# jcmgray/cotengra

Measured on NVIDIA H100. Metric: sycamore_n53_m20_sliced_contract_tflops, higher is better.
Workload: dtype c128 (f64 arithmetic)

## Files before the change

cotengra_b200/csrc/absorbdot.cuh:

```cuda
#pragma once

constexpr int AB_STAGES = 4;
constexpr int AB_THREADS = 256;
constexpr int AB_VSTAGE = 2 * 32 * 32;
constexpr int AB_ASTAGE = 2 * 32 * 16;
constexpr size_t AB_SMEM = (size_t)(128 * 16 + AB_STAGES * (AB_VSTAGE + AB_ASTAGE)) * sizeof(double2);

__device__ __forceinline__ double ab_neg(double x) { return __longlong_as_double(__double_as_longlong(x) ^ (1ll << 63)); }

__global__ void __launch_bounds__(AB_THREADS, 1)
absorbdot_kernel(const int64_t* __restrict__ D, const double2* __restrict__ A, const double2* __restrict__ Bs,
                 const double2* __restrict__ V, double2* __restrict__ C) {
  extern __shared__ __align__(16) double2 ab_smem[];
  double2* sB = ab_smem;
  double2* sV = sB + 128 * 16;
  double2* sA = sV + AB_STAGES * AB_VSTAGE;
  __shared__ long long t_ma[32], t_mc[32], t_nv[32], t_cv[128], t_ka[16];

  const int tid = threadIdx.x, lane = tid & 31, warp = tid >> 5;
  const int N = (int)D[AB_N], K = (int)D[AB_K], CC = (int)D[AB_C], CCP = (int)D[AB_CCP], KL = (int)D[AB_KL];
  const int NG = (int)D[AB_NG];
  const long long kla = D[AB_KLA], klv = D[AB_KLV];
  for (int i = tid; i < 32; i += AB_THREADS) {
    t_ma[i] = D[AB_TMA + i];
    t_mc[i] = D[AB_TMC + i];
    t_nv[i] = D[AB_TNV + i];
  }
  for (int i = tid; i < 128; i += AB_THREADS) t_cv[i] = D[AB_TCV + i];
  for (int i = tid; i < 16; i += AB_THREADS) t_ka[i] = D[AB_TKA + i];
  for (int i = tid; i < 128 * 16; i += AB_THREADS) {
    const int c = i >> 4, k = i & 15;
    const long long cb = D[AB_TCB + c];
    const bool ok = cb >= 0 && k < K;
    cp_async_zfill<16>(sB + c * 16 + (k ^ ((c & 1) << 2)), ok ? Bs + D[AB_TKB + k] + cb : Bs, ok);
  }
  __syncthreads();

  const unsigned long long U = (unsigned long long)D[AB_UNITS];
  const unsigned u0 = (unsigned)(U * blockIdx.x / gridDim.x), u1 = (unsigned)(U * (blockIdx.x + 1) / gridDim.x);
  const int nq = CCP >> 5;
  const long long nstage = (long long)(u1 - u0) * nq;

  unsigned g_ext = 1, g_div = 1;
  long long g_sa = 0, g_sv = 0;
  if (lane < NG) {
    g_ext = (unsigned)D[AB_G + lane * 4];
    g_div = (unsigned)D[AB_G + lane * 4 + 1];
    g_sa = D[AB_G + lane * 4 + 2];
    g_sv = D[AB_G + lane * 4 + 3];
  }
  auto unit_base = [&](unsigned u, long long& oa, long long& ov) {
    const long long dgt = (long long)((u / g_div) % g_ext);
    long long a = dgt * g_sa, v = dgt * g_sv;
#pragma unroll
    for (int o = 16; o > 0; o >>= 1) {
      a += __shfl_xor_sync(0xffffffffu, a, o);
      v += __shfl_xor_sync(0xffffffffu, v, o);
    }
    oa = a;
    ov = v;
  };

  unsigned lu = u0;
  int lq = 0;
  long long la = 0, lv = 0;
  if (nstage > 0) unit_base(lu, la, lv);
  long long issued = 0;
  auto issue = [&]() {
    if (issued < nstage) {
      const int slot = (int)(issued % AB_STAGES);
      double2* dv = sV + slot * AB_VSTAGE;
      double2* da = sA + slot * AB_ASTAGE;
#pragma unroll
      for (int j = 0; j < 8; ++j) {
        const int e = j * AB_THREADS + tid, cq = e & 31, kl = (e >> 5) & 1, n = e >> 6, c = lq * 32 + cq;
        const bool ok = kl < KL && n < N && c < CC;
        cp_async_zfill<16>(dv + (kl * 32 + n) * 32 + (cq ^ (n & 1)), ok ? V + lv + kl * klv + t_nv[n] + t_cv[c] : V, ok);
      }
#pragma unroll
      for (int j = 0; j < 4; ++j) {
        const int e = j * AB_THREADS + tid, k = e & 15, kl = (e >> 4) & 1, m = e >> 5;
        const bool ok = k < K && kl < KL && t_mc[m] >= 0;
        cp_async_zfill<16>(da + (kl * 32 + m) * 16 + (k ^ ((m & 1) << 2)), ok ? A + la + kl * kla + t_ka[k] + t_ma[m] : A,
                           ok);
      }
      ++issued;
      if (++lq == nq) {
        lq = 0;
        ++lu;
        if (issued < nstage) unit_base(lu, la, lv);
      }
    }
    cp_async_commit();
  };
#pragma unroll 1
  for (int s = 0; s < AB_STAGES - 1; ++s) issue();

  const int g = lane >> 2, t = lane & 3;
  const int wmh = warp >> 2, wcb = warp & 3;
  int bofs[2];
#pragma unroll
  for (int i = 0; i < 2; ++i) bofs[i] = (int)D[AB_TBCK + 2 * wmh + i] * CCP * 16;
  double Rr[4][2][2], Ri[4][2][2];
#pragma unroll
  for (int nb = 0; nb < 4; ++nb)
#pragma unroll
    for (int i = 0; i < 2; ++i) Rr[nb][i][0] = Rr[nb][i][1] = Ri[nb][i][0] = Ri[nb][i][1] = 0.0;

#pragma unroll 1
  for (long long s = 0; s < nstage; ++s) {
    cp_async_wait<AB_STAGES - 2>();
    __syncthreads();
    issue();
    const int slot = (int)(s % AB_STAGES), q = (int)(s % nq);
    if (q * 32 + wcb * 8 >= CC) continue;
    const double2* vb = sB + (q * 32 + wcb * 8 + g) * 16;
#pragma unroll
    for (int kl = 0; kl < 2; ++kl) {
      if (kl >= KL) break;
      const double2* va = sA + slot * AB_ASTAGE + (kl * 32 + wmh * 16) * 16;
      const double2* vv = sV + slot * AB_VSTAGE + kl * 32 * 32;
      double Xr[2][2], Xi[2][2];
#pragma unroll
      for (int i = 0; i < 2; ++i) Xr[i][0] = Xr[i][1] = Xi[i][0] = Xi[i][1] = 0.0;
#pragma unroll
      for (int ks = 0; ks < 4; ++ks) {
        const int kk = (ks * 4 + t) ^ ((g & 1) << 2);
#pragma unroll
        for (int i = 0; i < 2; ++i) {
          const double2 b = vb[bofs[i] + kk];
          const double2 a = va[(i * 8 + g) * 16 + kk];
          dmma16x8x4(Xr[i], Xi[i], a.x, a.y, b.x);
          dmma16x8x4(Xr[i], Xi[i], ab_neg(a.y), a.x, b.y);
        }
      }
#pragma unroll
      for (int p = 0; p < 2; ++p) {
#pragma unroll
        for (int nb = 0; nb < 4; ++nb) {
          const double2 v = vv[(nb * 8 + g) * 32 + ((wcb * 8 + 2 * t + p) ^ (g & 1))];
          const double nvi = ab_neg(v.y);
#pragma unroll
          for (int i = 0; i < 2; ++i) {
            dmma16x8x4(Rr[nb][i], Ri[nb][i], v.x, v.y, Xr[i][p]);
            dmma16x8x4(Rr[nb][i], Ri[nb][i], nvi, v.x, Xi[i][p]);
          }
        }
      }
    }
  }
  cp_async_wait<0>();
  __syncthreads();

  double2* red = sV;
#pragma unroll
  for (int nb = 0; nb < 4; ++nb)
#pragma unroll
    for (int i = 0; i < 2; ++i)
#pragma unroll
      for (int e = 0; e < 2; ++e)
        red[wcb * 1024 + ((2 * wmh + i) * 8 + 2 * t + e) * 32 + nb * 8 + g] = make_double2(Rr[nb][i][e], Ri[nb][i][e]);
  __syncthreads();
  for (int i = tid; i < 1024; i += AB_THREADS) {
    const int m = i >> 5, n = i & 31;
    if (t_mc[m] < 0 || n >= N) continue;
    double2 sum = red[i];
#pragma unroll
    for (int w = 1; w < 4; ++w) sum = add_of(sum, red[w * 1024 + i]);
    atomic_add_of(C + t_mc[m] + D[AB_TNC + n], sum);
  }
}
```

cotengra_b200/csrc/ctg_b200.cu:

```cuda
#include <cuda.h>
#include <cuda_runtime.h>
#include <stdint.h>
#include <stdio.h>
#include <stdlib.h>
#include <string.h>

#include <algorithm>
#include <atomic>
#include <type_traits>
#include <string>
#include <vector>

#include "../../include/ctg_b200.h"
#include "gett_desc.h"
#include "gett_kernels.cuh"
#include "probe.cuh"

using namespace ctgb;

namespace {

thread_local std::string g_err;
std::atomic<int64_t> g_launches{0};

// ... 233 lines not shown
  if (!di.ok) return fail(CTGB_E_CUDA, "no CUDA device");
  DsLaunch lc;
  if (int rc = dmmastream_launch_config(h, di.sms, lc)) return rc;
  if (lc.blocks == 0) return CTGB_OK;
  const bool strip = desc_stripped(h);
  const double2 *a = (const double2*)A, *b = (const double2*)B;
  double2* c = (double2*)C;
  const unsigned blocks = (unsigned)lc.blocks;
  switch (lc.nj) {
    case 1: dmmastream_launch<1, 4>(strip, blocks, d, a, b, c, st); break;
    case 2: dmmastream_launch<2, 4>(strip, blocks, d, a, b, c, st); break;
    case 4: dmmastream_launch<4, 4>(strip, blocks, d, a, b, c, st); break;
    default: dmmastream_launch<8, 2>(strip, blocks, d, a, b, c, st); break;
  }
  g_launches.fetch_add(1, std::memory_order_relaxed);
  CUDA_TRY(cudaGetLastError());
  return CTGB_OK;
}

int launch_absorb_root(const int64_t* h, const int64_t* d, const void* A, const void* Bs, const void* V, void* C,
                       cudaStream_t st) {
  if (h[W_DTYPE] != CTGB_C128) return fail(CTGB_E_VALUE, "the absorb-root kernel is complex128 only");
  if (h[AB_M] < 1 || h[AB_M] > 32 || h[AB_N] < 1 || h[AB_N] > 32 || h[AB_K] < 1 || h[AB_K] > 16 || h[AB_C] < 1 ||
      h[AB_C] > h[AB_CCP] || h[AB_CCP] % 32 || h[AB_CCP] > 128 || (h[AB_KL] != 1 && h[AB_KL] != 2) || h[AB_NG] < 0 || h[AB_NG] > AB_MAXG || h[AB_UNITS] < 1 || h[AB_UNITS] >= (1ll << 32) ||
      h[AB_GRID] < 1 || h[AB_GRID] > h[AB_UNITS] || h[AB_GRID] > (1 << 20))
    return fail(CTGB_E_VALUE, "absorb-root descriptor out of range");
  for (int mb = 0; mb < 4; ++mb)
    if (h[AB_TBCK + mb] < 0 || (h[AB_TBCK + mb] + 1) * h[AB_CCP] > 128)
      return fail(CTGB_E_VALUE, "absorb-root descriptor out of range");
  if (!(h[W_FLAGS] & 1)) {
    if (h[W_CELEMS] <= 0) return fail(CTGB_E_VALUE, "absorb-root into a strided C needs accumulate");
    CUDA_TRY(cudaMemsetAsync(C, 0, (size_t)h[W_CELEMS] * sizeof(double2), st));
  }
  static bool attr = false;
  if (!attr) {
    CUDA_TRY(cudaFuncSetAttribute(absorbdot_kernel, cudaFuncAttributeMaxDynamicSharedMemorySize, (int)AB_SMEM));
    attr = true;
  }
  absorbdot_kernel<<<(unsigned)h[AB_GRID], AB_THREADS, AB_SMEM, st>>>(d, (const double2*)A, (const double2*)Bs,
                                                                      (const double2*)V, (double2*)C);
  g_launches.fetch_add(1, std::memory_order_relaxed);
  CUDA_TRY(cudaGetLastError());
  return CTGB_OK;
}

std::atomic<int64_t> g_tmap_launches{0};

struct Tc05Box {
  int nb = 0;
  struct Dim { uint64_t ext, stride; } dim[8];
};
int tc05_tensor_map_box(const int64_t* h, uint64_t a_addr, Tc05Box& bx) {
  if (a_addr & 15u) return 0;
  auto& box = bx.dim;
  int& nb = bx.nb;
  nb = 0;
  const int n_lda = (int)h[W_NLDA];
  for (int i = 0; i < n_lda; ++i) {
    const uint64_t ext = (uint64_t)h[OFF_LDA + 4 * i], st = (uint64_t)h[OFF_LDA + 4 * i + 1];
    if (h[OFF_LDA + 4 * i + 1] <= 0) return 0;
    if (nb && st == box[nb - 1].stride * box[nb - 1].ext) {
      box[nb - 1].ext *= ext;
    } else {
      if (nb == 4) return 0;
      box[nb].ext = ext;
      box[nb].stride = st;
      ++nb;
    }
  }
  for (int i = 0; i < nb; ++i) {
    while (box[i].ext > 256) {
      uint64_t f = 256;
      while (f > 1 && box[i].ext % f) --f;
// ... 1074 lines not shown
```

cotengra_b200/executor.py:

```python

from __future__ import annotations

import ctypes as C
import math

import numpy as np

from . import _lib, lowering
from .lowering import (
    DTYPE_CODES,
    DTYPE_SIZES,
    accumulator_dtype,
    build_pair_desc,
    build_single_desc,
    check_precision,
    check_tensordot_shapes,
    classify_pair,
    classify_single,
    dtype_name,
    row_major_strides,
    split_equation,
    tensordot_terms,
)

# ... 199 lines not shown
        if self.acc_dtype not in (None, self.dtype):
            _lib.check(lib.ctgb_plan_set_accumulator(h, DTYPE_CODES[self.acc_dtype]))
        if self.scale_slots is not None:
            n = len(self.nodes)
            sa, sb = ((C.c_int32 * max(n, 1))(*s) for s in self.scale_slots)
            _lib.check(lib.ctgb_plan_set_scale_slots(h, sa, sb, n))
        return self

    def destroy(self):
        if self.handle is not None:
            _lib.load().ctgb_plan_destroy(self.handle)
            self.handle = None

    def launches_per_slice(self):
        return int(_lib.load().ctgb_plan_launches_per_slice(self.handle))

    def strip_modes(self):
        n = len(self.nodes)
        pre, after = (C.c_int32 * n)(), (C.c_int32 * n)()
        _lib.check(_lib.load().ctgb_plan_strip_modes(self.handle, pre, after, n))
        return [(int(a), int(b)) for a, b in zip(pre, after)]

    def __del__(self):
        try:
            self.destroy()
        except Exception:
            pass


class ExecPlan(_DevicePlan):

    def __init__(self, contractions, inputs, output, size_dict, sliced=(), dtype="complex128",
                 strip_exponent=False, hoist=True, allow_dmma=True, sm_count=None,
                 variant=None, precision="3xtf32", accumulate="native", absorb_root=False):
        self.dtype = dtype_name(dtype)
        self.precision = check_precision(precision, self.dtype)
        self.esize = DTYPE_SIZES[self.dtype]
        self.acc_dtype = accumulator_dtype(self.dtype, accumulate)
        self.wide = self.acc_dtype != self.dtype
        self.contractions = tuple(contractions)
        self.inputs = [tuple(t) for t in inputs]
        self.output = tuple(output)
        self.size_dict = dict(size_dict)
        self.sliced = [(i, int(s), None if p is None else int(p)) for i, s, p in sliced]
        self.strip_exponent = bool(strip_exponent)
        if sm_count is None:
            try:
                sm_count = _lib.device_info()["sm_count"]
            except Exception:
                sm_count = 132
        self.sm_count = sm_count
        self.absorb_root = bool(absorb_root) and self.dtype == "complex128" and not self.strip_exponent \
            and variant is None
        self._build(hoist, allow_dmma, variant)

    def _build(self, hoist, allow_dmma, variant):
        sliced_pos = {ind: j for j, (ind, _s, _p) in enumerate(self.sliced)}
        nslices = math.prod(s for _i, s, p in self.sliced if p is None)
        self.nslices = nslices
        real_slicing = bool(self.sliced)
        hoist = hoist and real_slicing

        def out_ext(ix):
            if ix in sliced_pos and self.sliced[sliced_pos[ix]][2] is not None:
                return 1
            return self.size_dict[ix]

        self.out_shape = tuple(out_ext(ix) for ix in self.output)
        out_full_strides = row_major_strides(self.out_shape)
        self.out_elements = math.prod(self.out_shape)
        root_term = tuple(ix for ix in self.output if ix not in sliced_pos)
        root_strides = [s for ix, s in zip(self.output, out_full_strides) if ix not in sliced_pos]
        self.root_shape = tuple(self.size_dict[ix] for ix in root_term)
        self.slice_out_stride = [0] * len(self.sliced)
        for ix, s in zip(self.output, out_full_strides):
            if ix in sliced_pos and self.sliced[sliced_pos[ix]][2] is None:
                self.slice_out_stride[sliced_pos[ix]] += s

        cur = {}
        self.input_nbytes = []
        for i, term in enumerate(self.inputs):
            full_shape = [self.size_dict[ix] for ix in term]
            fs = row_major_strides(full_shape)
            self.input_nbytes.append(math.prod(full_shape) * self.esize)
            keep = [k for k, ix in enumerate(term) if ix not in sliced_pos]
            cut = [k for k, ix in enumerate(term) if ix in sliced_pos]
            cur[i] = _Slot([full_shape[k] for k in keep], [fs[k] for k in keep], K_INPUT, self.input_nbytes[-1],
# ... 11 lines not shown
                terms, out = split_equation(arg)
                if len(terms) != 1:
                    raise ValueError(f"expected a single-term equation, got {arg!r}")
                is_root = l is not None
                if is_root and not is_last:
                    raise ValueError("single-input record must be the only contraction")
                ostr = root_strides if (is_root and direct) else None
                odims, sdims, oshape = classify_single(terms[0], src.shape, out, out_strides=ostr,
                                                      strides_x=src.strides)
                if is_root:
                    self._check_root_shape(oshape)
                acc = is_root and direct
                words = build_single_desc(odims, sdims, self.dtype, accumulate=acc)
                dst = _Slot(oshape, row_major_strides(oshape), K_SCRATCH, max(math.prod(oshape), 1) * self.esize,
                            variant=src.variant)
                nodes.append(dict(kind=1, a=src, b=None, c=dst, words=words, root=is_root))
                tensors.append(dst)
                cur[p] = dst
                continue

            A, Bt = cur.pop(l), cur.pop(r)
            if tdot:
                axes = (tuple(arg[0]), tuple(arg[1]))
                check_tensordot_shapes(axes, A.shape, Bt.shape)
                ta, tb, to = tensordot_terms(axes, len(A.shape), len(Bt.shape), perm)
            else:
                terms, to = split_equation(arg)
                if len(terms) != 2:
                    raise ValueError(f"expected a two-term equation, got {arg!r}")
                ta, tb = terms
            is_root = is_last

            def lower(into_output, wide_c=False):
                ostr = root_strides if into_output else None
                dims = classify_pair(ta, A.shape, tb, Bt.shape, to, out_strides=ostr,
                                     strides_a=A.strides, strides_b=Bt.strides)
                dense = 0 if into_output else math.prod(dims.out_shape)
                return dims, dense, build_pair_desc(dims, self.dtype, accumulate=into_output,
                                                    sm_count=self.sm_count, allow_dmma=allow_dmma,
                                                    c_dense_elems=dense, variant=variant,
                                                    precision=self.precision, wide_c=wide_c)

            if is_root and self.wide and not self.strip_exponent:
                direct = lower(True)[2].variant in lowering.DOTSTREAM_VARIANTS
                dims, dense, plan = lower(direct, wide_c=direct)
            else:
                dims, dense, plan = lower(is_root and direct)
            if is_root:
                self._check_root_shape(dims.out_shape)
            acc = is_root and direct
            dst = _Slot(dims.out_shape, row_major_strides(dims.out_shape), K_SCRATCH,
                        max(math.prod(dims.out_shape), 1) * self.esize, variant=A.variant or Bt.variant)
            a, b = (Bt, A) if plan.swapped else (A, Bt)
            nodes.append(dict(kind=0, a=a, b=b, c=dst, words=plan.words, root=is_root, plan=plan,
                              sizes=plan.sizes, dims=dims, acc=acc, dense=dense, terms=(A, Bt)))
            tensors.append(dst)
            cur[p] = dst
            if self.absorb_root:
                self._absorb(nodes, tensors)

        if not nodes:
            raise ValueError("empty contraction program")
        self.root_direct = direct
        if direct:
            nodes[-1]["c"].kind = K_OUTPUT
        for nd in nodes:
            srcs = [t for t in (nd["a"], nd["b"], nd.get("d")) if t is not None]
            nd["invariant"] = bool(hoist and not nd["root"] and not any(s.variant for s in srcs))
            nd["phase"] = PHASE_INV_FWD if nd["invariant"] else PHASE_VAR_FWD
            if nd["invariant"]:
                nd["c"].kind = K_PERSISTENT
            else:
                nd["c"].variant = True
        order = [nd for nd in nodes if nd["invariant"]] + [nd for nd in nodes if not nd["invariant"]]
        for pos, nd in enumerate(order):
            nd["pos"] = pos
        self.workspace_bytes, self.persistent_bytes, _ = layout(order)
        self.nodes = nodes
        self.n_variant_nodes = sum(1 for nd in nodes if not nd["invariant"])

        self.macs_per_slice = 0
        self.macs_invariant = 0
        self.elements_per_slice = 0
        for nd in nodes:
            if nd["kind"] != 0:
                continue
            macs = nd["plan"].macs if nd.get("d") is not None else math.prod(nd["sizes"])
            el = sum(math.prod(nd[x].shape) for x in ("a", "b", "d", "c") if nd.get(x) is not None)
            if nd["invariant"]:
                self.macs_invariant += macs
            else:
                self.macs_per_slice += macs
                self.elements_per_slice += el

        self.tensors = tensors
        self._marshal()
        if not direct:
            rs = self.root_shape
            dense = row_major_strides(rs)
            odims = [[e, sx, so] for e, sx, so in zip(rs, dense, root_strides) if e != 1]
            self._chunk_words = build_single_desc(odims, [], self.dtype)

    def _absorb(self, nodes, tensors):
        if len(nodes) < 2:
            return
        P, R = nodes[-2], nodes[-1]
        if P["kind"] != 0 or R["kind"] != 0 or P.get("d") is not None or R["plan"].variant != lowering.VAR_DMMA_32x32:
            return
        X = P["c"]
        if X not in R["terms"]:
            return
        ab = lowering.build_absorb_desc(P["dims"], R["dims"], R["terms"][0] is X, accumulate=R["acc"],
                                        sm_count=self.sm_count, c_dense_elems=R["dense"])
        if ab is None:
            return
        pa, pb = P["terms"]
        small, big = (pa, pb) if ab.small_is_a else (pb, pa)
        V = R["terms"][1] if R["terms"][0] is X else R["terms"][0]
        tensors.remove(X)
        nodes[-2:] = [dict(kind=0, a=big, b=V, d=small, c=R["c"], words=ab.words, root=R["root"], plan=ab,
                           sizes=ab.sizes, dims=None, acc=R["acc"], dense=R["dense"], terms=None)]

    def _check_root_shape(self, shape):
        if tuple(shape) != tuple(self.root_shape):
            raise ValueError(
                f"contraction program produces shape {tuple(shape)}, "
                f"tree output expects {tuple(self.root_shape)}"
            )

    def host_staging_bytes(self):
        extra = _align(self.total_bytes) - self.total_bytes
        for n in self.input_nbytes:
            extra += _align(n)
        return extra + _align(self.out_elements * DTYPE_SIZES[self.acc_dtype]) + 512

    def execute(self, input_ptrs, out_ptr, exp_ptr, ws_ptr, ws_bytes, begin, step, count, stream=0):
        lib = _lib.load()
        arr = (C.c_void_p * len(input_ptrs))(*input_ptrs)
        _lib.check(lib.ctgb_plan_execute(self.handle, arr, out_ptr, exp_ptr, None, None, ws_ptr, ws_bytes,
                                         int(begin), int(step), int(count), stream))

    def execute_host(self, host_arrays, host_out, ws_ptr, ws_bytes, begin, step, count, stream=0):
        lib = _lib.load()
        ptrs = (C.c_void_p * len(host_arrays))(*[a.ctypes.data for a in host_arrays])
        nb = (C.c_int64 * len(host_arrays))(*[a.nbytes for a in host_arrays])
        exp = C.c_double(0.0)
        _lib.check(lib.ctgb_plan_execute_host(self.handle, ptrs, nb, host_out.ctypes.data,
                                              C.byref(exp), ws_ptr, ws_bytes, int(begin), int(step),
                                              int(count), stream))
        return exp.value

    def profile(self, enable=True):
        _lib.check(_lib.load().ctgb_plan_profile(self.handle, int(enable)))

# ... 6 lines not shown
```

cotengra_b200/lowering.py:

```python

from __future__ import annotations

import math
from collections import Counter, namedtuple
from dataclasses import dataclass, field

import numpy as np

MAX_T, MAX_G, MAX_GB, MAX_LD = 12, 40, 12, 24
(W_MAGIC, W_DTYPE, W_NTM, W_NTN, W_NTK, W_NGM, W_NGN, W_NGK, W_NGB, W_MTA,
 W_NTA, W_KTA, W_TILES_M, W_TILES_N, W_TILES_B, W_STEPS_K, W_SPLITK, W_PGM,
 W_MFULL, W_MTEXT, W_MW, W_PGN, W_NFULL, W_NTEXT, W_NW, W_PGK, W_KFULL,
 W_KTEXT, W_KW, W_NLDA, W_NLDB, W_FLAGS, W_VARIANT, W_CELEMS, W_RUNA, W_LBOPAD) = range(36)
W_HDR = 40
OFF_TM = W_HDR
OFF_TN = OFF_TM + MAX_T * 3
OFF_TK = OFF_TN + MAX_T * 3
OFF_GM = OFF_TK + MAX_T * 3
OFF_GN = OFF_GM + MAX_G * 4
OFF_GK = OFF_GN + MAX_G * 4
OFF_GB = OFF_GK + MAX_G * 4
OFF_LDA = OFF_GB + MAX_GB * 5
OFF_LDB = OFF_LDA + MAX_LD * 4
DESC_WORDS = OFF_LDB + MAX_LD * 4
# ... 555 lines not shown
    for off, rows, width in ((OFF_TM, t.tm, 3), (OFF_TN, t.tn, 3), (OFF_TK, t.tk, 3), (OFF_GM, t.gm, 4),
                             (OFF_GN, t.gn, 4), (OFF_GK, t.gk, 4), (OFF_GB, t.gb, 5), (OFF_LDA, t.lda, 4),
                             (OFF_LDB, t.ldb, 4)):
        for i, r in enumerate(rows):
            W[off + i * width: off + (i + 1) * width] = r
    return W




AB_M, AB_N, AB_K, AB_C, AB_KL, AB_NG, AB_UNITS, AB_KLA, AB_KLV, AB_GRID, AB_BS_SLOT, AB_CCP = range(2, 14)
AB_MAXG = 32
AB_TMA = W_HDR
AB_TMC, AB_TNV, AB_TNC = AB_TMA + 32, AB_TMA + 64, AB_TMA + 96
AB_TKA = AB_TMA + 128
AB_TKB = AB_TKA + 16
AB_TCB = AB_TKB + 16
AB_TCV = AB_TCB + 128
AB_G = AB_TCV + 128
AB_TBCK = AB_G + AB_MAXG * 4


@dataclass
class AbsorbPlan:

    words: np.ndarray
    small_is_a: bool
    sizes: tuple
    macs: int
    variant: int = VAR_ABSORB_ROOT
    swapped: bool = False
    splitk: int = 1
    tiles: int = 1


def _enum(dims, cols):
    out = [[0] for _ in cols]
    for d in dims:
        out = [[o + i * d[c] for i in range(d[0]) for o in lst] for lst, c in zip(out, cols)]
    return out


def build_absorb_desc(dp: PairDims, dr: PairDims, x_is_a, accumulate=False, sm_count=132, c_dense_elems=0):
    if dp.batch or dr.batch:
        return None
    xi = 1 if x_is_a else 2
    vi = 3 - xi
    r_keep = {d[xi]: (d[0], d[3]) for d in (dr.m if x_is_a else dr.n)}
    v_keep = [[d[0], d[vi], d[3]] for d in (dr.n if x_is_a else dr.m)]
    r_con = {d[xi]: (d[0], d[vi]) for d in dr.k}
    if len(r_con) != len(dr.k) or len(r_keep) != len(dr.m if x_is_a else dr.n):
        return None
    for small_is_a in (False, True):
        small = dp.m if small_is_a else dp.n
        big = dp.n if small_is_a else dp.m
        bi, si = (2, 1) if small_is_a else (1, 2)
        xdims = {d[3]: d for d in small + big}
        if not small or len(xdims) != len(small) + len(big) or set(xdims) != set(r_keep) | set(r_con):
            continue
        if any(xdims[x][0] != (r_keep.get(x) or r_con[x])[0] for x in xdims):
            continue
        small_x = {d[3] for d in small}
        rows = [[d[0], d[bi], r_keep[d[3]][1]] for d in big if d[3] in r_keep]
        ck = [[d[0], d[si], r_keep[d[3]][1]] for d in small if d[3] in r_keep]
        cc = sorted(([d[0], d[si], r_con[d[3]][1]] for d in small if d[3] in r_con), key=lambda d: d[2])
        kprime = [[d[0], d[bi], r_con[d[3]][1]] for d in big if d[3] in r_con]
        MX, CK = math.prod(d[0] for d in rows), math.prod(d[0] for d in ck)
        N, K, CC = math.prod(d[0] for d in v_keep), math.prod(d[0] for d in dp.k), math.prod(d[0] for d in cc)
        CCP = -(-CC // 32) * 32
        rows_per = 8 if CK > 1 else 32
        if MX > rows_per or CK * rows_per > 32 or N > 32 or K > 16 or CK * CCP > 128 or not small_x:
            return None
        kl = min(kprime, key=lambda d: d[2], default=None)
        if kl is not None and kl[0] == 2:
            kprime.remove(kl)
        else:
            kl = [1, 0, 0]
        grid = sorted(kprime, key=lambda d: (d[1], d[2]))
        if len(grid) > AB_MAXG:
            return None
        units = math.prod(d[0] for d in grid)
        w = np.zeros(DESC_WORDS, dtype=np.int64)
        w[0], w[1] = DESC_MAGIC, DTYPE_CODES["complex128"]
        w[AB_M], w[AB_N], w[AB_K], w[AB_C], w[AB_CCP], w[AB_KL] = CK * rows_per if CK > 1 else MX, N, K, CC, CCP, kl[0]
        w[AB_NG], w[AB_UNITS], w[AB_KLA], w[AB_KLV] = len(grid), units, kl[1], kl[2]
        w[AB_GRID] = min(units, sm_count)
        w[AB_BS_SLOT] = -1
        w[W_FLAGS] = int(bool(accumulate))
        w[W_VARIANT] = VAR_ABSORB_ROOT
        w[W_CELEMS] = c_dense_elems
        ra, rc = _enum(rows, (1, 2))
        ckb, ckc = _enum(ck, (1, 2))
        ma, mc = [-1] * 32, [-1] * 32
        for j, (ob, oc) in enumerate(zip(ckb, ckc)):
            for r, (a, c) in enumerate(zip(ra, rc)):
                ma[j * rows_per + r], mc[j * rows_per + r] = a, c + oc
        tbck = [min(mb * 8 // rows_per, CK - 1) for mb in range(4)]
        nv, nc = _enum(v_keep, (1, 2))
        ka, kb = _enum([[d[0], d[bi], d[si]] for d in dp.k], (1, 2))
        cb, cv = _enum(cc, (1, 2))
        tcb = [-1] * 128
        for j, ob in enumerate(ckb):
            tcb[j * CCP:j * CCP + CC] = [ob + o for o in cb]
        for off, vals in ((AB_TMA, ma), (AB_TMC, mc), (AB_TNV, nv), (AB_TNC, nc), (AB_TKA, ka), (AB_TKB, kb),
                          (AB_TCB, tcb), (AB_TCV, cv), (AB_TBCK, tbck)):
            w[off:off + len(vals)] = vals
        div = 1
        for j, (e, sa, sv) in enumerate(grid):
            w[AB_G + 4 * j:AB_G + 4 * j + 4] = (e, div, sa, sv)
            div *= e
        kp = units * kl[0]
        M = MX * CK
        return AbsorbPlan(w, small_is_a, (1, M, N, kp * CC), MX * kp * K * CC * CK + M * N * kp * CC)
    return None


def classify_single(term, shape, out, out_strides=None, strides_x=None):
    term, out = tuple(term), tuple(out)
    shape = tuple(map(int, shape))
    if len(term) != len(shape):
        raise ValueError(f"Term '{term}' does not match shape {shape}.")
    sx = row_major_strides(shape) if strides_x is None else list(strides_x)
    ext, st_x, order = {}, {}, []
    for ix, d, s in zip(term, shape, sx):
        if ix not in order:
            order.append(ix)
        if ext.setdefault(ix, d) != d:
            raise ValueError(f"Index {ix} has mismatched sizes {ext[ix]} and {d}.")
        st_x[ix] = st_x.get(ix, 0) + s
    for ix in out:
        if ix not in ext:
            raise ValueError(f"Output index {ix} does not appear in the input.")
    out_shape = tuple(ext[ix] for ix in out)
    so = row_major_strides(out_shape) if out_strides is None else list(out_strides)
    odims = [[ext[ix], st_x[ix], s] for ix, s in zip(out, so) if ext[ix] != 1]
    sdims = [[ext[ix], st_x[ix]] for ix in order if ix not in out and ext[ix] != 1]
    return odims, sdims, out_shape


def build_single_desc(odims, sdims, dtype, accumulate=False) -> np.ndarray:
    dtype = dtype_name(dtype)
    odims = coalesce(odims)
    sdims = coalesce(sdims)
    odims.sort(key=lambda d: abs(d[2]) if d[2] else 1 << 62)
    sdims.sort(key=lambda d: abs(d[1]) if d[1] else 1 << 62)
    if len(odims) > MAX_S or len(sdims) > MAX_S:
        raise NotImplementedError("too many dims for a single-operand node")
# ... 26 lines not shown
```

cotengra_b200/csrc/gett_kernels.cuh:

```cuda
#pragma once
#include <cuda_runtime.h>
#include <math_constants.h>
#include <stdint.h>

#include <type_traits>

#include "gett_desc.h"

namespace ctgb {

__device__ __forceinline__ void mac(float& c, float a, float b) { c = fmaf(a, b, c); }
__device__ __forceinline__ void mac(double& c, double a, double b) { c = fma(a, b, c); }
__device__ __forceinline__ void mac(float2& c, float2 a, float2 b) {
  c.x = fmaf(a.x, b.x, c.x);
  c.x = fmaf(-a.y, b.y, c.x);
  c.y = fmaf(a.x, b.y, c.y);
  c.y = fmaf(a.y, b.x, c.y);
}
__device__ __forceinline__ void mac(double2& c, double2 a, double2 b) {
  c.x = fma(a.x, b.x, c.x);
  c.x = fma(-a.y, b.y, c.x);
  c.y = fma(a.x, b.y, c.y);
  c.y = fma(a.y, b.x, c.y);
}
// ... 497 lines not shown
    for (int i = 0; i < FM; ++i)
#pragma unroll
      for (int j = 0; j < FN; ++j) {
        if constexpr (TR) {
          const int r = (wm * FM + i) * 8 + fc;
          const int c = (wn * FN + j) * 8 + frow;
          store(r, c, make_double2(acc.re[i][j][0], acc.im[i][j][0]));
          store(r + 1, c, make_double2(acc.re[i][j][1], acc.im[i][j][1]));
          continue;
        }
        const int r = (wm * FM + i) * 8 + frow;
        const int c = (wn * FN + j) * 8 + fc;
        if constexpr (CPLX) {
          if (pair_ok) {
            store_pair(r, c, make_double2(acc.re[i][j][0], acc.im[i][j][0]),
                       make_double2(acc.re[i][j][1], acc.im[i][j][1]));
          } else {
            store(r, c, make_double2(acc.re[i][j][0], acc.im[i][j][0]));
            store(r, c + 1, make_double2(acc.re[i][j][1], acc.im[i][j][1]));
          }
        } else {
          store(r, c, acc.re[i][j][0]);
          store(r, c + 1, acc.re[i][j][1]);
        }
      }
  }
};

#include "tf32_policy.cuh"
#include "stream_rows.cuh"
#include "rowstream.cuh"
#include "dmmastream.cuh"
#include "dotstream.cuh"
#include "absorbdot.cuh"
#include "tc05_policy.cuh"
#include "gett_ws.cuh"
#include "tc05_kernel.cuh"

template <typename T>
__global__ void single_kernel(const int64_t* __restrict__ D, const T* __restrict__ X, T* __restrict__ out) {
  const int n_o = (int)D[S_NO], n_s = (int)D[S_NS];
  const long long out_elems = D[S_OUT_ELEMS], sum_elems = D[S_SUM_ELEMS];
  const bool accumulate = (D[S_FLAGS] & 1) != 0;
  for (long long o = blockIdx.x * (long long)blockDim.x + threadIdx.x; o < out_elems;
       o += (long long)gridDim.x * blockDim.x) {
    long long e = o, xo = 0, oo = 0;
    for (int d = 0; d < n_o; ++d) {
      const int64_t* L = D + OFF_SO + d * 3;
      long long dig = e % L[0];
      e /= L[0];
      xo += dig * L[1];
      oo += dig * L[2];
    }
    T acc = zero_of<T>();
    for (long long s = 0; s < sum_elems; ++s) {
      long long e2 = s, xs = 0;
      for (int d = 0; d < n_s; ++d) {
        const int64_t* L = D + OFF_SS + d * 2;
        xs += (e2 % L[0]) * L[1];
        e2 /= L[0];
      }
      acc = add_of(acc, X[xo + xs]);
    }
    out[oo] = accumulate ? add_of(out[oo], acc) : acc;
  }
}

template <typename T>
__global__ void __launch_bounds__(256) single_reduce_kernel(const int64_t* __restrict__ D, const T* __restrict__ X,
// ... 182 lines not shown
```

Baseline: 24.38.

## Template absorb-root kernel on row count and add optional block-friendly root layout

The absorb-root kernel is now templated on whether the A rows collapse to 8 unique rows. When they do, it loads a smaller A tile per stage and uses a deeper 5-stage cp.async ring. The host checks the row tables to pick the instantiation. Separately, a new opt-in root_layout option rewrites the output strides of the producer steps feeding the absorbed root, so A and V arrive in a block-friendly bit order. That option is off by default and adds a second build pass when enabled.

```diff
diff --git a/cotengra_b200/csrc/absorbdot.cuh b/cotengra_b200/csrc/absorbdot.cuh
--- a/cotengra_b200/csrc/absorbdot.cuh
+++ b/cotengra_b200/csrc/absorbdot.cuh
@@ -1,16 +1,23 @@
 #pragma once
 
-constexpr int AB_STAGES = 4;
 constexpr int AB_THREADS = 256;
 constexpr int AB_VSTAGE = 2 * 32 * 32;
-constexpr int AB_ASTAGE = 2 * 32 * 16;
-constexpr size_t AB_SMEM = (size_t)(128 * 16 + AB_STAGES * (AB_VSTAGE + AB_ASTAGE)) * sizeof(double2);
+template <bool ROWS8>
+struct AbRing {
+  static constexpr int STAGES = ROWS8 ? 5 : 4;
+  static constexpr int AROWS = ROWS8 ? 8 : 32;
+  static constexpr int ASTAGE = 2 * AROWS * 16;
+  static constexpr size_t SMEM = (size_t)(128 * 16 + STAGES * (AB_VSTAGE + ASTAGE)) * sizeof(double2);
+};
+static_assert(AbRing<true>::SMEM <= 232448 && AbRing<false>::SMEM <= 232448, "absorb-root ring fits shared memory");
 
 __device__ __forceinline__ double ab_neg(double x) { return __longlong_as_double(__double_as_longlong(x) ^ (1ll << 63)); }
 
+template <bool ROWS8>
 __global__ void __launch_bounds__(AB_THREADS, 1)
 absorbdot_kernel(const int64_t* __restrict__ D, const double2* __restrict__ A, const double2* __restrict__ Bs,
                  const double2* __restrict__ V, double2* __restrict__ C) {
+  constexpr int AB_STAGES = AbRing<ROWS8>::STAGES, AB_AROWS = AbRing<ROWS8>::AROWS, AB_ASTAGE = AbRing<ROWS8>::ASTAGE;
   extern __shared__ __align__(16) double2 ab_smem[];
   double2* sB = ab_smem;
   double2* sV = sB + 128 * 16;
@@ -78,11 +85,11 @@
         cp_async_zfill<16>(dv + (kl * 32 + n) * 32 + (cq ^ (n & 1)), ok ? V + lv + kl * klv + t_nv[n] + t_cv[c] : V, ok);
       }
 #pragma unroll
-      for (int j = 0; j < 4; ++j) {
+      for (int j = 0; j < AB_AROWS / 8; ++j) {
         const int e = j * AB_THREADS + tid, k = e & 15, kl = (e >> 4) & 1, m = e >> 5;
         const bool ok = k < K && kl < KL && t_mc[m] >= 0;
-        cp_async_zfill<16>(da + (kl * 32 + m) * 16 + (k ^ ((m & 1) << 2)), ok ? A + la + kl * kla + t_ka[k] + t_ma[m] : A,
-                           ok);
+        cp_async_zfill<16>(da + (kl * AB_AROWS + m) * 16 + (k ^ ((m & 1) << 2)),
+                           ok ? A + la + kl * kla + t_ka[k] + t_ma[m] : A, ok);
       }
       ++issued;
       if (++lq == nq) {
@@ -118,7 +125,7 @@
 #pragma unroll
     for (int kl = 0; kl < 2; ++kl) {
       if (kl >= KL) break;
-      const double2* va = sA + slot * AB_ASTAGE + (kl * 32 + wmh * 16) * 16;
+      const double2* va = sA + slot * AB_ASTAGE + (kl * AB_AROWS + (ROWS8 ? 0 : wmh * 16)) * 16;
       const double2* vv = sV + slot * AB_VSTAGE + kl * 32 * 32;
       double Xr[2][2], Xi[2][2];
 #pragma unroll
@@ -129,7 +136,7 @@
 #pragma unroll
         for (int i = 0; i < 2; ++i) {
           const double2 b = vb[bofs[i] + kk];
-          const double2 a = va[(i * 8 + g) * 16 + kk];
+          const double2 a = va[((ROWS8 ? 0 : i * 8) + g) * 16 + kk];
           dmma16x8x4(Xr[i], Xi[i], a.x, a.y, b.x);
           dmma16x8x4(Xr[i], Xi[i], ab_neg(a.y), a.x, b.y);
         }
diff --git a/cotengra_b200/csrc/ctg_b200.cu b/cotengra_b200/csrc/ctg_b200.cu
--- a/cotengra_b200/csrc/ctg_b200.cu
+++ b/cotengra_b200/csrc/ctg_b200.cu
@@ -289,13 +289,22 @@
     if (h[W_CELEMS] <= 0) return fail(CTGB_E_VALUE, "absorb-root into a strided C needs accumulate");
     CUDA_TRY(cudaMemsetAsync(C, 0, (size_t)h[W_CELEMS] * sizeof(double2), st));
   }
-  static bool attr = false;
-  if (!attr) {
-    CUDA_TRY(cudaFuncSetAttribute(absorbdot_kernel, cudaFuncAttributeMaxDynamicSharedMemorySize, (int)AB_SMEM));
-    attr = true;
-  }
-  absorbdot_kernel<<<(unsigned)h[AB_GRID], AB_THREADS, AB_SMEM, st>>>(d, (const double2*)A, (const double2*)Bs,
-                                                                      (const double2*)V, (double2*)C);
+  bool rows8 = true;
+  for (int r = 8; r < 32; ++r)
+    if (h[AB_TMC + r] >= 0 && (h[AB_TMC + (r & 7)] < 0 || h[AB_TMA + r] != h[AB_TMA + (r & 7)])) rows8 = false;
+  static bool attr[2] = {false, false};
+  if (!attr[rows8]) {
+    CUDA_TRY(cudaFuncSetAttribute(rows8 ? absorbdot_kernel<true> : absorbdot_kernel<false>,
+                                  cudaFuncAttributeMaxDynamicSharedMemorySize,
+                                  (int)(rows8 ? AbRing<true>::SMEM : AbRing<false>::SMEM)));
+    attr[rows8] = true;
+  }
+  if (rows8)
+    absorbdot_kernel<true><<<(unsigned)h[AB_GRID], AB_THREADS, AbRing<true>::SMEM, st>>>(
+        d, (const double2*)A, (const double2*)Bs, (const double2*)V, (double2*)C);
+  else
+    absorbdot_kernel<false><<<(unsigned)h[AB_GRID], AB_THREADS, AbRing<false>::SMEM, st>>>(
+        d, (const double2*)A, (const double2*)Bs, (const double2*)V, (double2*)C);
   g_launches.fetch_add(1, std::memory_order_relaxed);
   CUDA_TRY(cudaGetLastError());
   return CTGB_OK;
diff --git a/cotengra_b200/executor.py b/cotengra_b200/executor.py
--- a/cotengra_b200/executor.py
+++ b/cotengra_b200/executor.py
@@ -255,7 +255,7 @@
 
     def __init__(self, contractions, inputs, output, size_dict, sliced=(), dtype="complex128",
                  strip_exponent=False, hoist=True, allow_dmma=True, sm_count=None,
-                 variant=None, precision="3xtf32", accumulate="native", absorb_root=False):
+                 variant=None, precision="3xtf32", accumulate="native", absorb_root=False, root_layout=False):
         self.dtype = dtype_name(dtype)
         self.precision = check_precision(precision, self.dtype)
         self.esize = DTYPE_SIZES[self.dtype]
@@ -275,7 +275,15 @@
         self.sm_count = sm_count
         self.absorb_root = bool(absorb_root) and self.dtype == "complex128" and not self.strip_exponent \
             and variant is None
+        self._out_strides, self._cc_order = {}, None
         self._build(hoist, allow_dmma, variant)
+        self.root_layout = False
+        if root_layout and self.absorb_root:
+            lay = self._root_block_layout()
+            if lay is not None:
+                self._out_strides, self._cc_order = lay
+                self.root_layout = True
+                self._build(hoist, allow_dmma, variant)
 
     def _build(self, hoist, allow_dmma, variant):
         sliced_pos = {ind: j for j, (ind, _s, _p) in enumerate(self.sliced)}
@@ -353,7 +361,7 @@
             is_root = is_last
 
             def lower(into_output, wide_c=False):
-                ostr = root_strides if into_output else None
+                ostr = root_strides if into_output else self._out_strides.get(step)
                 dims = classify_pair(ta, A.shape, tb, Bt.shape, to, out_strides=ostr,
                                      strides_a=A.strides, strides_b=Bt.strides)
                 dense = 0 if into_output else math.prod(dims.out_shape)
@@ -370,11 +378,11 @@
             if is_root:
                 self._check_root_shape(dims.out_shape)
             acc = is_root and direct
-            dst = _Slot(dims.out_shape, row_major_strides(dims.out_shape), K_SCRATCH,
+            dst = _Slot(dims.out_shape, self._out_strides.get(step, row_major_strides(dims.out_shape)), K_SCRATCH,
                         max(math.prod(dims.out_shape), 1) * self.esize, variant=A.variant or Bt.variant)
             a, b = (Bt, A) if plan.swapped else (A, Bt)
             nodes.append(dict(kind=0, a=a, b=b, c=dst, words=plan.words, root=is_root, plan=plan,
-                              sizes=plan.sizes, dims=dims, acc=acc, dense=dense, terms=(A, Bt)))
+                              sizes=plan.sizes, dims=dims, acc=acc, dense=dense, terms=(A, Bt), step=step))
             tensors.append(dst)
             cur[p] = dst
             if self.absorb_root:
@@ -432,7 +440,7 @@
         if X not in R["terms"]:
             return
         ab = lowering.build_absorb_desc(P["dims"], R["dims"], R["terms"][0] is X, accumulate=R["acc"],
-                                        sm_count=self.sm_count, c_dense_elems=R["dense"])
+                                        sm_count=self.sm_count, c_dense_elems=R["dense"], cc_order=self._cc_order)
         if ab is None:
             return
         pa, pb = P["terms"]
@@ -441,6 +449,19 @@
         tensors.remove(X)
         nodes[-2:] = [dict(kind=0, a=big, b=V, d=small, c=R["c"], words=ab.words, root=R["root"], plan=ab,
                            sizes=ab.sizes, dims=None, acc=R["acc"], dense=R["dense"], terms=None)]
+
+    def _root_block_layout(self):
+        F = next((nd for nd in self.nodes if nd.get("d") is not None), None)
+        if F is None:
+            return None
+        writer = {id(nd["c"]): nd for nd in self.nodes if nd["kind"] == 0 and nd.get("d") is None}
+        wa, wv = writer.get(id(F["a"])), writer.get(id(F["b"]))
+        if wa is None or wv is None:
+            return None
+        st = lowering.absorb_block_strides(F["plan"], F["a"].shape, F["a"].strides, F["b"].shape, F["b"].strides)
+        if st is None:
+            return None
+        return {wa["step"]: st[0], wv["step"]: st[1]}, [d[2] for d in F["plan"].roles["cc"]]
 
     def _check_root_shape(self, shape):
         if tuple(shape) != tuple(self.root_shape):
diff --git a/cotengra_b200/lowering.py b/cotengra_b200/lowering.py
--- a/cotengra_b200/lowering.py
+++ b/cotengra_b200/lowering.py
@@ -611,6 +611,7 @@
     swapped: bool = False
     splitk: int = 1
     tiles: int = 1
+    roles: dict = None
 
 
 def _enum(dims, cols):
@@ -620,7 +621,8 @@
     return out
 
 
-def build_absorb_desc(dp: PairDims, dr: PairDims, x_is_a, accumulate=False, sm_count=132, c_dense_elems=0):
+def build_absorb_desc(dp: PairDims, dr: PairDims, x_is_a, accumulate=False, sm_count=132, c_dense_elems=0,
+                      cc_order=None):
     if dp.batch or dr.batch:
         return None
     xi = 1 if x_is_a else 2
@@ -642,7 +644,8 @@
         small_x = {d[3] for d in small}
         rows = [[d[0], d[bi], r_keep[d[3]][1]] for d in big if d[3] in r_keep]
         ck = [[d[0], d[si], r_keep[d[3]][1]] for d in small if d[3] in r_keep]
-        cc = sorted(([d[0], d[si], r_con[d[3]][1]] for d in small if d[3] in r_con), key=lambda d: d[2])
+        cc = sorted(([d[0], d[si], r_con[d[3]][1], d[3]] for d in small if d[3] in r_con),
+                    key=(lambda d: d[2]) if cc_order is None else (lambda d: cc_order.index(d[3])))
         kprime = [[d[0], d[bi], r_con[d[3]][1]] for d in big if d[3] in r_con]
         MX, CK = math.prod(d[0] for d in rows), math.prod(d[0] for d in ck)
         N, K, CC = math.prod(d[0] for d in v_keep), math.prod(d[0] for d in dp.k), math.prod(d[0] for d in cc)
@@ -690,8 +693,34 @@
             div *= e
         kp = units * kl[0]
         M = MX * CK
-        return AbsorbPlan(w, small_is_a, (1, M, N, kp * CC), MX * kp * K * CC * CK + M * N * kp * CC)
+        roles = dict(rows=[d[:2] for d in rows], k=[[d[0], d[bi]] for d in dp.k],
+                     cc=[[d[0], d[2], d[3]] for d in cc], n=[d[:2] for d in v_keep], kl=kl, grid=grid)
+        return AbsorbPlan(w, small_is_a, (1, M, N, kp * CC), MX * kp * K * CC * CK + M * N * kp * CC,
+                          roles=roles)
     return None
+
+
+def absorb_block_strides(ab: AbsorbPlan, shape_a, strides_a, shape_v, strides_v):
+    ro = ab.roles
+    if ro is None or ro["kl"][0] != 2 or [len(ro[r]) for r in ("rows", "k", "cc", "n")] != [3, 4, 5, 5]:
+        return None
+    if any(d[0] != 2 for r in ("rows", "k", "cc", "n", "grid") for d in ro[r]):
+        return None
+    if any(e != 2 for e in tuple(shape_a) + tuple(shape_v)):
+        return None
+    m, k, c, n, kl, grid = ro["rows"], ro["k"], ro["cc"], ro["n"], ro["kl"], ro["grid"]
+    va = [k[0], k[1], m[0], k[2], k[3], m[1], m[2], kl] + grid
+    vv = [c[1], c[2], n[0], c[0], c[3], c[4], n[1], n[2], n[3], n[4], [2, kl[2]]] + [[2, g[2]] for g in grid]
+    out = []
+    for order, shape, strides in ((va, shape_a, strides_a), (vv, shape_v, strides_v)):
+        pos = {s: i for i, s in enumerate(strides)}
+        if len(order) != len(shape) or len(pos) != len(strides) or {d[1] for d in order} != set(pos):
+            return None
+        new = [0] * len(shape)
+        for bit, d in enumerate(order):
+            new[pos[d[1]]] = 1 << bit
+        out.append(new)
+    return tuple(out)
 
 
 def classify_single(term, shape, out, out_strides=None, strides_x=None):
```

Result: faster. 24.73 (median of 6 runs) (+1.4%).

## Warp-specialize absorb-root kernel with mbarrier producer ring and specialized variants

Applied to the files above, without the earlier changes.

Converts the absorb-root DMMA kernel from a cp.async multistage loop with block-wide syncs into a warp-specialized design. Four producer warps fill a shared-memory ring tracked by full/empty mbarriers, and eight consumer warps compute, with registers rebalanced between the two groups. Template variants are added: one dedups A rows when rows 8-31 repeat rows 0-7, which shrinks each A stage and allows a fifth stage; the other keeps B fragments in registers when CCP is 32. The aim is to remove __syncthreads stalls and shared-memory traffic, at the cost of extra threads, more register pressure, and four kernel instantiations.

```diff
diff --git a/cotengra_b200/csrc/absorbdot.cuh b/cotengra_b200/csrc/absorbdot.cuh
--- a/cotengra_b200/csrc/absorbdot.cuh
+++ b/cotengra_b200/csrc/absorbdot.cuh
@@ -1,26 +1,33 @@
 #pragma once
 
-constexpr int AB_STAGES = 4;
-constexpr int AB_THREADS = 256;
+constexpr int AB_CONSUMERS = 256;
+constexpr int AB_THREADS = AB_CONSUMERS + 128;
 constexpr int AB_VSTAGE = 2 * 32 * 32;
-constexpr int AB_ASTAGE = 2 * 32 * 16;
-constexpr size_t AB_SMEM = (size_t)(128 * 16 + AB_STAGES * (AB_VSTAGE + AB_ASTAGE)) * sizeof(double2);
+
+template <bool A8>
+struct AbRing {
+  static constexpr int AROWS = A8 ? 8 : 32;
+  static constexpr int ASTAGE = 2 * AROWS * 16;
+  static constexpr int STAGES = A8 ? 5 : 4;
+  static constexpr size_t SMEM = (size_t)(128 * 16 + STAGES * (AB_VSTAGE + ASTAGE)) * sizeof(double2);
+};
 
 __device__ __forceinline__ double ab_neg(double x) { return __longlong_as_double(__double_as_longlong(x) ^ (1ll << 63)); }
 
+template <bool A8, bool BREG>
 __global__ void __launch_bounds__(AB_THREADS, 1)
 absorbdot_kernel(const int64_t* __restrict__ D, const double2* __restrict__ A, const double2* __restrict__ Bs,
                  const double2* __restrict__ V, double2* __restrict__ C) {
+  using RG = AbRing<A8>;
   extern __shared__ __align__(16) double2 ab_smem[];
   double2* sB = ab_smem;
   double2* sV = sB + 128 * 16;
-  double2* sA = sV + AB_STAGES * AB_VSTAGE;
+  double2* sA = sV + RG::STAGES * AB_VSTAGE;
   __shared__ long long t_ma[32], t_mc[32], t_nv[32], t_cv[128], t_ka[16];
+  __shared__ unsigned long long bar_full[RG::STAGES], bar_empty[RG::STAGES];
 
   const int tid = threadIdx.x, lane = tid & 31, warp = tid >> 5;
   const int N = (int)D[AB_N], K = (int)D[AB_K], CC = (int)D[AB_C], CCP = (int)D[AB_CCP], KL = (int)D[AB_KL];
-  const int NG = (int)D[AB_NG];
-  const long long kla = D[AB_KLA], klv = D[AB_KLV];
   for (int i = tid; i < 32; i += AB_THREADS) {
     t_ma[i] = D[AB_TMA + i];
     t_mc[i] = D[AB_TMC + i];
@@ -34,6 +41,15 @@
     const bool ok = cb >= 0 && k < K;
     cp_async_zfill<16>(sB + c * 16 + (k ^ ((c & 1) << 2)), ok ? Bs + D[AB_TKB + k] + cb : Bs, ok);
   }
+  if (tid == 0) {
+    for (int s = 0; s < RG::STAGES; ++s) {
+      mbar_init(&bar_full[s], AB_THREADS - AB_CONSUMERS);
+      mbar_init(&bar_empty[s], AB_CONSUMERS / 32);
+    }
+    asm volatile("fence.mbarrier_init.release.cluster;\n" ::: "memory");
+  }
+  cp_async_commit();
+  cp_async_wait<0>();
   __syncthreads();
 
   const unsigned long long U = (unsigned long long)D[AB_UNITS];
@@ -41,116 +57,150 @@
   const int nq = CCP >> 5;
   const long long nstage = (long long)(u1 - u0) * nq;
 
-  unsigned g_ext = 1, g_div = 1;
-  long long g_sa = 0, g_sv = 0;
-  if (lane < NG) {
-    g_ext = (unsigned)D[AB_G + lane * 4];
-    g_div = (unsigned)D[AB_G + lane * 4 + 1];
-    g_sa = D[AB_G + lane * 4 + 2];
-    g_sv = D[AB_G + lane * 4 + 3];
-  }
-  auto unit_base = [&](unsigned u, long long& oa, long long& ov) {
-    const long long dgt = (long long)((u / g_div) % g_ext);
-    long long a = dgt * g_sa, v = dgt * g_sv;
-#pragma unroll
-    for (int o = 16; o > 0; o >>= 1) {
-      a += __shfl_xor_sync(0xffffffffu, a, o);
-      v += __shfl_xor_sync(0xffffffffu, v, o);
-    }
-    oa = a;
-    ov = v;
-  };
-
-  unsigned lu = u0;
-  int lq = 0;
-  long long la = 0, lv = 0;
-  if (nstage > 0) unit_base(lu, la, lv);
-  long long issued = 0;
-  auto issue = [&]() {
-    if (issued < nstage) {
-      const int slot = (int)(issued % AB_STAGES);
-      double2* dv = sV + slot * AB_VSTAGE;
-      double2* da = sA + slot * AB_ASTAGE;
-#pragma unroll
-      for (int j = 0; j < 8; ++j) {
-        const int e = j * AB_THREADS + tid, cq = e & 31, kl = (e >> 5) & 1, n = e >> 6, c = lq * 32 + cq;
-        const bool ok = kl < KL && n < N && c < CC;
-        cp_async_zfill<16>(dv + (kl * 32 + n) * 32 + (cq ^ (n & 1)), ok ? V + lv + kl * klv + t_nv[n] + t_cv[c] : V, ok);
-      }
-#pragma unroll
-      for (int j = 0; j < 4; ++j) {
-        const int e = j * AB_THREADS + tid, k = e & 15, kl = (e >> 4) & 1, m = e >> 5;
-        const bool ok = k < K && kl < KL && t_mc[m] >= 0;
-        cp_async_zfill<16>(da + (kl * 32 + m) * 16 + (k ^ ((m & 1) << 2)), ok ? A + la + kl * kla + t_ka[k] + t_ma[m] : A,
-                           ok);
-      }
-      ++issued;
+  if (warp >= AB_CONSUMERS / 32) {
+    reg_dealloc<56>();
+    const int pw = warp - AB_CONSUMERS / 32;
+    const int NG = (int)D[AB_NG];
+    const long long kla = D[AB_KLA], klv = D[AB_KLV];
+    unsigned g_ext = 1, g_div = 1;
+    long long g_sa = 0, g_sv = 0;
+    if (lane < NG) {
+      g_ext = (unsigned)D[AB_G + lane * 4];
+      g_div = (unsigned)D[AB_G + lane * 4 + 1];
+      g_sa = D[AB_G + lane * 4 + 2];
+      g_sv = D[AB_G + lane * 4 + 3];
+    }
+    auto unit_base = [&](unsigned u, long long& oa, long long& ov) {
+      const long long dgt = (long long)((u / g_div) % g_ext);
+      long long a = dgt * g_sa, v = dgt * g_sv;
+#pragma unroll
+      for (int o = 16; o > 0; o >>= 1) {
+        a += __shfl_xor_sync(0xffffffffu, a, o);
+        v += __shfl_xor_sync(0xffffffffu, v, o);
+      }
+      oa = a;
+      ov = v;
+    };
+    const int vkl = (lane >> 1) & 1, vc = (lane & 1) | ((lane >> 2) << 1);
+    const int akl = lane >> 4, ak = lane & 15;
+    unsigned lu = u0;
+    int lq = 0;
+    long long la = 0, lv = 0;
+    unit_base(lu, la, lv);
+    int slot = 0;
+    unsigned ph = 0;
+#pragma unroll 1
+    for (long long s = 0; s < nstage; ++s) {
+      mbar_wait(&bar_empty[slot], ph ^ 1);
+      double2* dv = sV + slot * AB_VSTAGE + vkl * 32 * 32;
+      double2* da = sA + slot * RG::ASTAGE + akl * RG::AROWS * 16;
+#pragma unroll
+      for (int h = 0; h < 2; ++h) {
+        const int cq = vc + 16 * h, c = lq * 32 + cq;
+        const bool okc = vkl < KL && c < CC;
+        const double2* src = V + lv + vkl * klv + t_cv[c];
+#pragma unroll
+        for (int n = 8 * pw; n < 8 * pw + 8; ++n) {
+          const bool ok = okc && n < N;
+          cp_async_zfill<16>(dv + n * 32 + (cq ^ (n & 1)), ok ? src + t_nv[n] : V, ok);
+        }
+      }
+      {
+        const bool okk = ak < K && akl < KL;
+        const double2* src = A + la + akl * kla + t_ka[ak];
+#pragma unroll
+        for (int m = pw; m < RG::AROWS; m += 4) {
+          const bool ok = okk && t_mc[m] >= 0;
+          cp_async_zfill<16>(da + m * 16 + (ak ^ ((m & 1) << 2)), ok ? src + t_ma[m] : A, ok);
+        }
+      }
+      mbar_arrive_cp_async(&bar_full[slot]);
+      if (++slot == RG::STAGES) {
+        slot = 0;
+        ph ^= 1;
+      }
       if (++lq == nq) {
         lq = 0;
         ++lu;
-        if (issued < nstage) unit_base(lu, la, lv);
+        if (s + 1 < nstage) unit_base(lu, la, lv);
       }
     }
     cp_async_commit();
-  };
-#pragma unroll 1
-  for (int s = 0; s < AB_STAGES - 1; ++s) issue();
-
+    cp_async_wait<0>();
+    return;
+  }
+
+  reg_alloc<224>();
   const int g = lane >> 2, t = lane & 3;
   const int wmh = warp >> 2, wcb = warp & 3;
   int bofs[2];
 #pragma unroll
   for (int i = 0; i < 2; ++i) bofs[i] = (int)D[AB_TBCK + 2 * wmh + i] * CCP * 16;
+  double2 breg[2][4];
+  if constexpr (BREG) {
+#pragma unroll
+    for (int i = 0; i < 2; ++i)
+#pragma unroll
+      for (int ks = 0; ks < 4; ++ks) breg[i][ks] = sB[(wcb * 8 + g) * 16 + bofs[i] + ((ks * 4 + t) ^ ((g & 1) << 2))];
+  }
   double Rr[4][2][2], Ri[4][2][2];
 #pragma unroll
   for (int nb = 0; nb < 4; ++nb)
 #pragma unroll
     for (int i = 0; i < 2; ++i) Rr[nb][i][0] = Rr[nb][i][1] = Ri[nb][i][0] = Ri[nb][i][1] = 0.0;
 
+  int slot = 0, q = 0;
+  unsigned ph = 0;
 #pragma unroll 1
   for (long long s = 0; s < nstage; ++s) {
-    cp_async_wait<AB_STAGES - 2>();
-    __syncthreads();
-    issue();
-    const int slot = (int)(s % AB_STAGES), q = (int)(s % nq);
-    if (q * 32 + wcb * 8 >= CC) continue;
-    const double2* vb = sB + (q * 32 + wcb * 8 + g) * 16;
-#pragma unroll
-    for (int kl = 0; kl < 2; ++kl) {
-      if (kl >= KL) break;
-      const double2* va = sA + slot * AB_ASTAGE + (kl * 32 + wmh * 16) * 16;
-      const double2* vv = sV + slot * AB_VSTAGE + kl * 32 * 32;
-      double Xr[2][2], Xi[2][2];
-#pragma unroll
-      for (int i = 0; i < 2; ++i) Xr[i][0] = Xr[i][1] = Xi[i][0] = Xi[i][1] = 0.0;
-#pragma unroll
-      for (int ks = 0; ks < 4; ++ks) {
-        const int kk = (ks * 4 + t) ^ ((g & 1) << 2);
-#pragma unroll
-        for (int i = 0; i < 2; ++i) {
-          const double2 b = vb[bofs[i] + kk];
-          const double2 a = va[(i * 8 + g) * 16 + kk];
-          dmma16x8x4(Xr[i], Xi[i], a.x, a.y, b.x);
-          dmma16x8x4(Xr[i], Xi[i], ab_neg(a.y), a.x, b.y);
-        }
-      }
-#pragma unroll
-      for (int p = 0; p < 2; ++p) {
-#pragma unroll
-        for (int nb = 0; nb < 4; ++nb) {
-          const double2 v = vv[(nb * 8 + g) * 32 + ((wcb * 8 + 2 * t + p) ^ (g & 1))];
-          const double nvi = ab_neg(v.y);
+    mbar_wait(&bar_full[slot], ph);
+    if (q * 32 + wcb * 8 < CC) {
+      const double2* vb = sB + (q * 32 + wcb * 8 + g) * 16;
+#pragma unroll
+      for (int kl = 0; kl < 2; ++kl) {
+        if (kl >= KL) break;
+        const double2* va = sA + slot * RG::ASTAGE + kl * RG::AROWS * 16 + (A8 ? 0 : wmh * 16 * 16);
+        const double2* vv = sV + slot * AB_VSTAGE + kl * 32 * 32;
+        double Xr[2][2], Xi[2][2];
+#pragma unroll
+        for (int i = 0; i < 2; ++i) Xr[i][0] = Xr[i][1] = Xi[i][0] = Xi[i][1] = 0.0;
+#pragma unroll
+        for (int ks = 0; ks < 4; ++ks) {
+          const int kk = (ks * 4 + t) ^ ((g & 1) << 2);
+          double2 a[2];
+          a[0] = va[g * 16 + kk];
+          a[1] = A8 ? a[0] : va[(8 + g) * 16 + kk];
 #pragma unroll
           for (int i = 0; i < 2; ++i) {
-            dmma16x8x4(Rr[nb][i], Ri[nb][i], v.x, v.y, Xr[i][p]);
-            dmma16x8x4(Rr[nb][i], Ri[nb][i], nvi, v.x, Xi[i][p]);
+            const double2 b = BREG ? breg[i][ks] : vb[bofs[i] + kk];
+            dmma16x8x4(Xr[i], Xi[i], a[i].x, a[i].y, b.x);
+            dmma16x8x4(Xr[i], Xi[i], ab_neg(a[i].y), a[i].x, b.y);
           }
         }
-      }
-    }
-  }
-  cp_async_wait<0>();
-  __syncthreads();
+#pragma unroll
+        for (int p = 0; p < 2; ++p) {
+#pragma unroll
+          for (int nb = 0; nb < 4; ++nb) {
+            const double2 v = vv[(nb * 8 + g) * 32 + ((wcb * 8 + 2 * t + p) ^ (g & 1))];
+            const double nvi = ab_neg(v.y);
+#pragma unroll
+            for (int i = 0; i < 2; ++i) {
+              dmma16x8x4(Rr[nb][i], Ri[nb][i], v.x, v.y, Xr[i][p]);
+              dmma16x8x4(Rr[nb][i], Ri[nb][i], nvi, v.x, Xi[i][p]);
+            }
+          }
+        }
+      }
+    }
+    __syncwarp();
+    if (lane == 0) mbar_arrive(&bar_empty[slot]);
+    if (++slot == RG::STAGES) {
+      slot = 0;
+      ph ^= 1;
+    }
+    if (++q == nq) q = 0;
+  }
+  named_sync<1, AB_CONSUMERS>();
 
   double2* red = sV;
 #pragma unroll
@@ -160,8 +210,8 @@
 #pragma unroll
       for (int e = 0; e < 2; ++e)
         red[wcb * 1024 + ((2 * wmh + i) * 8 + 2 * t + e) * 32 + nb * 8 + g] = make_double2(Rr[nb][i][e], Ri[nb][i][e]);
-  __syncthreads();
-  for (int i = tid; i < 1024; i += AB_THREADS) {
+  named_sync<1, AB_CONSUMERS>();
+  for (int i = tid; i < 1024; i += AB_CONSUMERS) {
     const int m = i >> 5, n = i & 31;
     if (t_mc[m] < 0 || n >= N) continue;
     double2 sum = red[i];
diff --git a/cotengra_b200/csrc/ctg_b200.cu b/cotengra_b200/csrc/ctg_b200.cu
--- a/cotengra_b200/csrc/ctg_b200.cu
+++ b/cotengra_b200/csrc/ctg_b200.cu
@@ -289,13 +289,21 @@
     if (h[W_CELEMS] <= 0) return fail(CTGB_E_VALUE, "absorb-root into a strided C needs accumulate");
     CUDA_TRY(cudaMemsetAsync(C, 0, (size_t)h[W_CELEMS] * sizeof(double2), st));
   }
-  static bool attr = false;
-  if (!attr) {
-    CUDA_TRY(cudaFuncSetAttribute(absorbdot_kernel, cudaFuncAttributeMaxDynamicSharedMemorySize, (int)AB_SMEM));
-    attr = true;
-  }
-  absorbdot_kernel<<<(unsigned)h[AB_GRID], AB_THREADS, AB_SMEM, st>>>(d, (const double2*)A, (const double2*)Bs,
-                                                                      (const double2*)V, (double2*)C);
+  bool a8 = true;
+  for (int r = 8; r < 32; ++r)
+    if (h[AB_TMC + r] >= 0 && (h[AB_TMC + r % 8] < 0 || h[AB_TMA + r] != h[AB_TMA + r % 8])) a8 = false;
+  const bool breg = h[AB_CCP] == 32;
+  using Kern = void (*)(const int64_t*, const double2*, const double2*, const double2*, double2*);
+  const Kern kern = a8 ? (breg ? absorbdot_kernel<true, true> : absorbdot_kernel<true, false>)
+                    : (breg ? absorbdot_kernel<false, true> : absorbdot_kernel<false, false>);
+  const size_t smem = a8 ? AbRing<true>::SMEM : AbRing<false>::SMEM;
+  static bool attr[4] = {};
+  if (!attr[2 * a8 + breg]) {
+    CUDA_TRY(cudaFuncSetAttribute(kern, cudaFuncAttributeMaxDynamicSharedMemorySize, (int)smem));
+    attr[2 * a8 + breg] = true;
+  }
+  kern<<<(unsigned)h[AB_GRID], AB_THREADS, smem, st>>>(d, (const double2*)A, (const double2*)Bs, (const double2*)V,
+                                                       (double2*)C);
   g_launches.fetch_add(1, std::memory_order_relaxed);
   CUDA_TRY(cudaGetLastError());
   return CTGB_OK;
diff --git a/cotengra_b200/csrc/gett_kernels.cuh b/cotengra_b200/csrc/gett_kernels.cuh
--- a/cotengra_b200/csrc/gett_kernels.cuh
+++ b/cotengra_b200/csrc/gett_kernels.cuh
@@ -553,9 +553,9 @@
 #include "rowstream.cuh"
 #include "dmmastream.cuh"
 #include "dotstream.cuh"
-#include "absorbdot.cuh"
 #include "tc05_policy.cuh"
 #include "gett_ws.cuh"
+#include "absorbdot.cuh"
 #include "tc05_kernel.cuh"
 
 template <typename T>
```

Result: faster. 24.48 before, 25.24 after (median of 6 runs) (+3.1%).
